# golmschenk/sr-gan

Hardware: AMD Instinct MI355X
Metric: SRGAN train images/sec (G+D step) (higher is better)
Workload: dtype f32; 1 GPU; crowd SRGAN (KnnDenseNetCat D/DNN + DCGenerator) 512x512, batch 16/GPU, dnn_training_step + gan_training_step per step; global_batch=16, image_size=512, schedule=shared-forwards, parallelism=dp1, random_init_weights=True, gradient_penalty=active, launch=eager (Python tape enqueues every kernel), schedule_check=not run: the --full option runs it

## Files before the change

include/srgan_hip.h:

```cpp
#ifndef SRGAN_HIP_H
#define SRGAN_HIP_H

#include <stdint.h>

#ifdef __cplusplus
extern "C" {
#endif

int srgan_version(void);
const char* srgan_build_id(void);
const char* srgan_last_error(void);

#define SRGAN_DTYPE_F32 0x1u
#define SRGAN_DTYPE_BF16 0x2u
#define SRGAN_DTYPE_F16 0x4u
#define SRGAN_FEATURE_FUSED_BNRELU 0x1u
#define SRGAN_FEATURE_SPLITK_WORKSPACE 0x2u
#define SRGAN_FEATURE_LIVE_PROFILE 0x4u
#define SRGAN_FEATURE_BLOCKED16 0x8u
#define SRGAN_FEATURE_BATCHED_SHADOWS 0x10u
#define SRGAN_FEATURE_CROWD_FULL_IMAGE 0x20u
#define SRGAN_FEATURE_IMAGE_BATCHES 0x40u
#define SRGAN_FEATURE_BATCH_NORM_TRAIN 0x80u
typedef struct srgan_capabilities_t {
// ... 31 lines not shown

int srgan_conv2d_bwd_weight(const srgan_conv_desc* desc, const float* x, const float* gy, float* gw, int accumulate,
                            int force_kernel, void* stream);

typedef struct srgan_bn_relu { const float* mean; const float* inv_std; const float* gamma; const float* beta; } srgan_bn_relu;
int srgan_conv2d_bnrelu_supported(const srgan_conv_desc* desc, int pass);
int srgan_conv2d_fwd_bnrelu(const srgan_conv_desc* desc, const float* x, const srgan_bn_relu* bn, const float* w,
                            const float* bias, float* y, void* stream);
int srgan_conv2d_fwd_bnrelu_splits(const srgan_conv_desc* desc);
int srgan_conv2d_fwd_bnrelu_into_zeros(const srgan_conv_desc* desc, const float* x, const srgan_bn_relu* bn, const float* w,
                                       const float* bias, float* y, void* stream);
int srgan_conv2d_bwd_data_bnrelu(const srgan_conv_desc* desc, const float* gy, const float* w, const srgan_bn_relu* bn,
                                 const float* x, float* gx, float* g_gamma, float* g_beta, int accumulate, void* stream);
int srgan_conv2d_bwd_weight_bnrelu(const srgan_conv_desc* desc, const float* x, const srgan_bn_relu* bn, const float* gy,
                                   float* gw, int accumulate, void* stream);
typedef struct srgan_bn_reduce_job {
  int64_t partial_offset;
  int32_t tiles, channels;
  const float* inv_std;
  float* g_gamma;
  float* g_beta;
} srgan_bn_reduce_job;
int64_t srgan_conv2d_bwd_data_bnrelu_tiles(const srgan_conv_desc* desc);
int srgan_conv2d_bwd_data_bnrelu_partials(const srgan_conv_desc* desc, const float* gy, const float* w, const srgan_bn_relu* bn,
                                          const float* x, float* gx, float* partials, int accumulate, void* stream);
int srgan_bn_partial_reduce_batched(const srgan_bn_reduce_job* jobs_device, int32_t count, int32_t max_channels, int32_t max_tiles,
                                    const float* scratch, void* stream);

int srgan_wgrad_group_plan(const srgan_conv_desc* desc, const srgan_bn_relu* bn, int64_t x_offset, int64_t gy_offset, float* gw,
                           int64_t gw_offset, int32_t group_size, int64_t group_weights, int64_t partial_offset, void* job,
// ... 185 lines not shown
```

sr-gan_amd/_lib.py:

```python
import ctypes
import os

from ._build import LIBRARY, source_id

c_float_p = ctypes.c_void_p
i32, i64, f32, vp = ctypes.c_int32, ctypes.c_int64, ctypes.c_float, ctypes.c_void_p


class ConvDesc(ctypes.Structure):
    _fields_ = [(name, i32) for name in ('N', 'C', 'H', 'W', 'K', 'R', 'S', 'stride_h', 'stride_w', 'pad_h', 'pad_w',
                                         'OH', 'OW')] + [('x_batch_stride', i64), ('y_batch_stride', i64), ('compute_dtype', i32)]


class BnRelu(ctypes.Structure):
    _fields_ = [(name, vp) for name in ('mean', 'inv_std', 'gamma', 'beta')]


class BnReduceJob(ctypes.Structure):
    _fields_ = [('partial_offset', i64), ('tiles', i32), ('channels', i32), ('inv_std', vp), ('g_gamma', vp), ('g_beta', vp)]


class Capabilities(ctypes.Structure):
    _fields_ = [('abi_version', i32), ('struct_bytes', i32), ('arch', ctypes.c_char * 16), ('dtypes', ctypes.c_uint32),
                ('features', ctypes.c_uint32), ('workspace_bytes', i64), ('max_tensor_elements', i64)]


SIGNATURES = {
    'srgan_version': ([], ctypes.c_int),
    'srgan_build_id': ([], ctypes.c_char_p),
    'srgan_last_error': ([], ctypes.c_char_p),
    'srgan_conv2d_fwd': ([ctypes.POINTER(ConvDesc), vp, vp, vp, vp, ctypes.c_int, vp], ctypes.c_int),
    'srgan_conv2d_bwd_data': ([ctypes.POINTER(ConvDesc), vp, vp, vp, vp, ctypes.c_int, ctypes.c_int, vp],
                              ctypes.c_int),
    'srgan_conv2d_bwd_weight': ([ctypes.POINTER(ConvDesc), vp, vp, vp, ctypes.c_int, ctypes.c_int, vp], ctypes.c_int),
    'srgan_conv2d_bnrelu_supported': ([ctypes.POINTER(ConvDesc), ctypes.c_int], ctypes.c_int),
    'srgan_conv2d_fwd_bnrelu': ([ctypes.POINTER(ConvDesc), vp, ctypes.POINTER(BnRelu), vp, vp, vp, vp], ctypes.c_int),
    'srgan_conv2d_fwd_bnrelu_into_zeros': ([ctypes.POINTER(ConvDesc), vp, ctypes.POINTER(BnRelu), vp, vp, vp, vp],
                                           ctypes.c_int),
    'srgan_conv2d_fwd_bnrelu_splits': ([ctypes.POINTER(ConvDesc)], ctypes.c_int),
    'srgan_bn_conv_tangent_weights': ([vp, vp, vp, vp, vp, vp, vp, i32, i32, i32, vp], ctypes.c_int),
    'srgan_conv2d_bwd_data_bnrelu': ([ctypes.POINTER(ConvDesc), vp, vp, ctypes.POINTER(BnRelu), vp, vp, vp, vp,
                                      ctypes.c_int, vp], ctypes.c_int),
    'srgan_conv2d_bwd_data_bnrelu_tiles': ([ctypes.POINTER(ConvDesc)], ctypes.c_int64),
    'srgan_conv2d_bwd_data_bnrelu_partials': ([ctypes.POINTER(ConvDesc), vp, vp, ctypes.POINTER(BnRelu), vp, vp, vp,
                                               ctypes.c_int, vp], ctypes.c_int),
    'srgan_bn_partial_reduce_batched': ([vp, i32, i32, i32, vp, vp], ctypes.c_int),
    'srgan_conv2d_bwd_weight_bnrelu': ([ctypes.POINTER(ConvDesc), vp, ctypes.POINTER(BnRelu), vp, vp, ctypes.c_int, vp],
                                       ctypes.c_int),
    'srgan_gemm_f32': ([i32, i32, i32, vp, i64, i64, vp, i64, i64, vp, i64, i64, vp, i32, ctypes.c_int, ctypes.c_int,
                        vp], ctypes.c_int),
    'srgan_gemm': ([i32, i32, i32, vp, i64, i64, vp, i64, i64, vp, i64, i64, vp, i32, ctypes.c_int, ctypes.c_int,
                    ctypes.c_int, vp], ctypes.c_int),
    'srgan_ew_unary': ([ctypes.c_int, vp, vp, i64, f32, f32, vp], ctypes.c_int),
    'srgan_ew_binary': ([ctypes.c_int, vp, vp, vp, i64, f32, vp], ctypes.c_int),
# ... 157 lines not shown
```

sr-gan_amd/csrc/gather_gemm_kernels.hip:

```cpp
#include "common.h"
#include "split_finish.h"
#include "gather_gemm.h"
#include "conv_plan.h"
#include "launchers.h"
#include <stdarg.h>
#include <string.h>
#include <stdlib.h>
#include <atomic>
#include <map>
#include <mutex>
#include <string>
#include <type_traits>
#include <type_traits>
#include <utility>

namespace srgan {

static thread_local char g_error[512] = "";

void set_error(const char* fmt, ...) {
  va_list ap;
  va_start(ap, fmt);
  vsnprintf(g_error, sizeof(g_error), fmt, ap);
  va_end(ap);
// ... 993 lines not shown
    if (pointwise(g)) return use_pointwise(g, g.K, 0) ? 1 : 0;
    return (use_conv3x3(g, g.K, 0) && g.C <= 512) ? 1 : 0;
  }
  if (pass == 1) {
    if ((size_t)g.N * g.H * g.W * g.C / 8 > WORKSPACE_BYTES) return 0;
    if (pointwise(g)) return use_pointwise(g, g.C, 0) ? 1 : 0;
    return (use_conv3x3(g, g.C, 0) && conv3x3_epilogue_supported(g.N, g.K, g.C, g.H, g.W)) ? 1 : 0;
  }
  if (pass == 2) {
    if (pointwise(g)) return pointwise_wgrad_geometry(g) ? 1 : 0;
    return wgrad3x3_geometry(g) ? 1 : 0;
  }
  return 0;
}

static int fwd_bnrelu(const srgan_conv_desc* desc, const float* x, const srgan_bn_relu* bn, const float* w, const float* bias,
                      float* y, int y_state, int* plan_only_split, void* stream) {
  ConvGeom g;
  SRGAN_GEOM(desc, g, "srgan_conv2d_fwd_bnrelu");
  SRGAN_REQUIRE(plan_only_split || (x && w && y && bn_ok(bn)), SRGAN_EINVAL, "srgan_conv2d_fwd_bnrelu pointers");
  SRGAN_REQUIRE(srgan_conv2d_bnrelu_supported(desc, 0), SRGAN_EUNSUPPORTED, "srgan_conv2d_fwd_bnrelu geometry support");
  const float* const coefficients[4] = {bn ? bn->mean : nullptr, bn ? bn->inv_std : nullptr, bn ? bn->gamma : nullptr,
                                        bn ? bn->beta : nullptr};
  if (pointwise(g) && (plan_only_split || ((uintptr_t)w & 15) == 0) &&
      pointwise_ksplit_wanted(g.N, g.C, g.K, g.H * g.W, true)) {
    if (plan_only_split) { *plan_only_split = 1; return SRGAN_OK; }
    return pointwise_ksplit_run(x, g.x_bs, w, bias, y, g.y_bs, g.N, g.C, g.K, g.H * g.W, 0, (hipStream_t)stream,
                                coefficients);
  }
  if (pointwise(g))
// ... 256 lines not shown
```

sr-gan_amd/csrc/launchers.h:

```cpp
#pragma once
#include "common.h"

namespace srgan {

int profile_bracket_begin(hipStream_t stream);
int profile_bracket_end(int slot, hipStream_t stream, int64_t M, int64_t N, int64_t K, int kind, int bm, int bn, int split,
                        int akf = 0, int bkf = 0, int64_t b_unique = 0, int precision = 0);
int profile_bracket_end_bytes(int slot, hipStream_t stream, int64_t M, int64_t N, int64_t K, int kind, int bm, int bn, int split,
                              double bytes, int precision);

struct Conv3Placement { int32_t taps, out_plane, out_sy, out_sx, out_off; };
int conv3x3_splits(int32_t N, int32_t CI, int32_t CO, int32_t H, int32_t W, int precision = 0);
bool conv3x3_epilogue_supported(int32_t N, int32_t CI, int32_t CO, int32_t H, int32_t W);
int64_t conv3x3_epilogue_tiles(int32_t N, int32_t CI, int32_t CO, int32_t H, int32_t W);
int conv3x3_run(const float* in, int64_t in_bs, const float* w, int32_t w_base, int32_t w_so, int32_t w_si, int32_t w_skh,
                int32_t w_skw, const float* bias, float* out, int64_t out_bs, int32_t N, int32_t CI, int32_t CO, int32_t H,
                int32_t W, int accumulate, hipStream_t stream, const float* const* bn = nullptr,
                const BnBackwardEpilogue* epilogue = nullptr, int precision = 0, const Conv3Placement* placement = nullptr);

constexpr int GROUP_OVERSUBSCRIPTION = 4;

int conv3x3_wgrad_run(const float* x, int64_t x_bs, const float* gy, int64_t gy_bs, float* gw, int32_t N, int32_t CI,
                      int32_t CO, int32_t H, int32_t W, int accumulate, hipStream_t stream, const float* const* bn = nullptr,
                      int precision = 0);
// ... 10 lines not shown
                  int* plan_only_split = nullptr);
int64_t pointwise_epilogue_tiles(int32_t N, int32_t HW);
void bn_partial_reduce_run(const float* partial, int tiles, int CO, const float* inv_std, float* g_gamma, float* g_beta,
                           hipStream_t stream);
int bn_partial_reduce_batched_run(const srgan_bn_reduce_job* jobs, int count, int max_channels, int max_tiles,
                                  const float* scratch, hipStream_t stream);

bool pointwise_ring_eligible(const float* in, int64_t in_bs, const float* w, int32_t w_so, int32_t w_si, const float* bias,
                             const float* out, int64_t out_bs, int32_t N, int32_t CI, int32_t CO, int32_t HW, bool fused_pro,
                             const BnBackwardEpilogue* epilogue, int* tile_pixels);
int pointwise_ring_run(const float* in, int64_t in_bs, const float* w, int32_t w_so, int32_t w_si, float* out, int64_t out_bs,
                       int32_t N, int32_t CI, int32_t CO, int32_t HW, int accumulate, hipStream_t stream,
                       const float* const* bn, const BnBackwardEpilogue* epilogue, float* epi_partial, int32_t epi_cols,
                       int tile_pixels, int32_t* rows_done);

bool pointwise_ksplit_wanted(int32_t N, int32_t K, int32_t M, int32_t HW, bool fused_bn);
int pointwise_ksplit_run(const float* in, int64_t in_bs, const float* w, const float* bias, float* out, int64_t out_bs,
                         int32_t N, int32_t K, int32_t M, int32_t HW, int accumulate, hipStream_t stream,
                         const float* const* bn);

bool pointwise_wgrad_enabled();
int pointwise_wgrad_run(const float* x, int64_t x_bs, const float* gy, int64_t gy_bs, float* gw, int32_t N, int32_t CI,
                        int32_t CO, int32_t HW, int accumulate, hipStream_t stream, const float* const* bn = nullptr);
int pointwise_wgrad_group_plan(int64_t x_off, int64_t x_bs, int64_t gy_off, int64_t gy_bs, float* gw, int64_t gw_off, int32_t N, int32_t CI,
                               int32_t CO, int32_t HW, const float* const* bn, int32_t group, int64_t group_weights, int64_t partial_offset,
                               void* job_out, int32_t* grid_x, int32_t* grid_y, int32_t* ragged, int64_t* partial_floats);
int pointwise_wgrad_group_run(const void* jobs, int32_t count, int32_t grid_x, int32_t grid_y, int32_t ragged, int32_t fused_bn,
                              const float* x_base, const float* gy_base, float* gw_base, int64_t flops_mn, int64_t pixels,
                              int64_t elements, int64_t partial_floats, hipStream_t stream);

// ... 22 lines not shown
```

sr-gan_amd/csrc/pointwise.hip:

```cpp
#include "common.h"
#include "launchers.h"
#include "split_finish.h"
#include <stdlib.h>
#include <type_traits>

namespace srgan {

typedef float f32x16 __attribute__((ext_vector_type(16)));

struct PointwiseParams {
  const float* in;
  const float* w;
  float* out;
  const float* bias;
  int32_t N, CI, CO, HW;
  int64_t in_bs, out_bs;
  int32_t w_so, w_si;
  int32_t gpi;
  int32_t tiles_m;
  int32_t xcd_remap;
  int32_t m_base;
  int32_t k_per_split;
  int32_t mode;
  float* split_ws;
// ... 549 lines not shown
  const int profile_slot = profile_bracket_begin(stream);
  p.xcd_remap = (p.tiles_m > 1 && blocks % 8 == 0) ? 1 : 0;
  const dim3 grid((unsigned)blocks, (unsigned)split, 1);
  if (mi == 2) launch_pointwise<2>(p, grid, stream);
  else launch_pointwise<1>(p, grid, stream);
  if (p.epi_partial && !epilogue->partial_out)
    bn_partial_reduce_run(p.epi_partial, (int)col_blocks, CO, p.bn_inv, epilogue->g_gamma, epilogue->g_beta, stream);
  const int status = launch_status();
  const int64_t pixels = (int64_t)N * HW;
  const int64_t b_elements = (int64_t)CI * pixels + (epilogue ? (int64_t)CO * pixels * (p.mode == 1 ? 2 : 1) : 0) +
                             ((!epilogue && p.mode == 1) ? (int64_t)CO * pixels : 0);
  profile_bracket_end(profile_slot, stream, CO, pixels, CI, 3, mi * 32, 128, split, 0, 0, b_elements);
  return status;
}

}
```

sr-gan_amd/csrc/pointwise_ring.hip:

```cpp
#include <atomic>
#include "common.h"
#include "launchers.h"
#include "lds_dma.h"
#include <stdlib.h>
#include <type_traits>

namespace srgan {

typedef float f32x16 __attribute__((ext_vector_type(16)));
typedef float f32x4 __attribute__((ext_vector_type(4)));
typedef float f32x2 __attribute__((ext_vector_type(2)));

struct RingParams {
  const float* in;
  const float* w;
  float* out;
  int32_t N, CI, CO, HW;
  int64_t in_bs, out_bs;
  int32_t w_ld;
  int32_t bpi;
  int32_t tiles_m;
  int32_t xcd_remap;
  int32_t mode;
  const float* bn_mean; const float* bn_inv; const float* bn_gamma; const float* bn_beta;
  const float* epi_x; int64_t epi_x_bs;
  float* epi_partial; int32_t epi_cols;
};

template <int STAGES, int NI, bool A_KCONTIG, int FUSE>
__global__ __launch_bounds__(256, 2) void pointwise_ring_kernel(const RingParams p) {
  constexpr int BK = 32;
  constexpr int A_BYTES = 128 * BK * 4, RB = 128 * NI, B_BYTES = BK * RB, C_BYTES = FUSE == 1 ? 4 * 512 : 0;
  constexpr int STAGE_BYTES = A_BYTES + B_BYTES + C_BYTES;
  constexpr int QA = 4, QB = NI, RPI = 1024 / RB;
  constexpr int PER_STAGE = QA + QB + (FUSE == 1 ? 2 : 0);
  static_assert(FUSE != 2 || NI == 4, "the epilogue's partial sums are per 128-pixel block");
  extern __shared__ __attribute__((aligned(16))) char smem[];
  const int tid = threadIdx.x, lane = tid & 63, l31 = lane & 31, lhi = lane >> 5;
  const int wave = __builtin_amdgcn_readfirstlane(tid >> 6);
  int bid = (int)blockIdx.x;
  if (p.xcd_remap) bid = (bid & 7) * ((int)gridDim.x >> 3) + (bid >> 3);
  const int tm = bid % p.tiles_m, cb = bid / p.tiles_m;
  const int n = cb / p.bpi, pix0 = (cb - n * p.bpi) * (32 * NI);
  const int m0 = tm * 128;
  const uint32_t lds0 = ring_lds_address(smem);
  const int nst = p.CI / BK;

  const char* in_block = (const char*)(p.in + (int64_t)n * p.in_bs + pix0);
  const int b_row = lane / (RB / 16), b_col = lane % (RB / 16);
  const uint32_t b_lane = (uint32_t)(b_row * p.HW + 4 * b_col) * 4u;
  uint32_t a_lane[QA];
  if (A_KCONTIG) {
#pragma unroll
    for (int q = 0; q < QA; ++q) {
      const int br = lane >> 4, sp = lane & 15;
      const int bank_row = 16 * wave + 4 * q + br;
      const int s = sp ^ (bank_row & 15);
      a_lane[q] = (uint32_t)(min(m0 + 2 * bank_row + (s >> 3), p.CO - 1) * p.w_ld + 4 * (s & 7)) * 4u;
    }
  } else {
#pragma unroll
    for (int q = 0; q < QA; ++q)
      a_lane[q] = (uint32_t)(((wave * QA + q) * 2 + lhi) * p.w_ld + min(m0 + 4 * l31, p.CO - 4)) * 4u;
  }
  const bool active = m0 + 32 * wave < p.CO;
  const float* c_lane0 = (lhi ? p.bn_inv : p.bn_mean) + l31;
  const float* c_lane1 = (lhi ? p.bn_beta : p.bn_gamma) + l31;
  auto issue = [&](int stage) {
    const uint32_t slot = lds0 + (uint32_t)(stage % STAGES) * STAGE_BYTES;
    const char* xb = in_block + (int64_t)(stage * BK + wave * QB * RPI) * p.HW * 4;
#pragma unroll
    for (int q = 0; q < QB; ++q)
      ring_glds16(xb + (int64_t)(q * RPI) * p.HW * 4, b_lane, slot + A_BYTES + (uint32_t)((wave * QB + q) * RPI) * RB);
    const char* wb = (const char*)p.w + (A_KCONTIG ? (int64_t)stage * BK * 4 : (int64_t)stage * BK * p.w_ld * 4);
#pragma unroll
    for (int q = 0; q < QA; ++q)
      ring_glds16(wb, a_lane[q], slot + (A_KCONTIG ? (uint32_t)(4096 * wave + 1024 * q) : (uint32_t)((wave * QA + q) * 1024)));
    if (FUSE == 1) {
      ring_glds4(c_lane0 + stage * BK, slot + A_BYTES + B_BYTES + wave * 512);
      ring_glds4(c_lane1 + stage * BK, slot + A_BYTES + B_BYTES + wave * 512 + 256);
    }
  };

  uint32_t a_read[4];
  if (A_KCONTIG) {
    const int row = 32 * wave + l31, bank_row = row >> 1;
#pragma unroll
    for (int g = 0; g < 4; ++g) a_read[g] = (uint32_t)(bank_row * 256 + ((((row & 1) * 8 + 2 * g + lhi) ^ (bank_row & 15)) * 16));
  } else {
#pragma unroll
    for (int g = 0; g < 4; ++g) a_read[g] = (uint32_t)((8 * g + 4 * lhi) * 512 + (32 * wave + l31) * 4);
  }
  const uint32_t b_read = (uint32_t)(A_BYTES + (4 * lhi) * RB + l31 * (4 * NI));
  const uint32_t c_read = (uint32_t)(A_BYTES + B_BYTES + wave * 512 + 16 * lhi);

  f32x16 acc[NI];
#pragma unroll
  for (int ni = 0; ni < NI; ++ni)
#pragma unroll
    for (int r = 0; r < 16; ++r) acc[ni][r] = 0.f;

  struct Group { float a[4]; float b[4][NI]; f32x4 mean, inv, gamma, beta; };
  auto load_group = [&](Group& f, const char* slot, int g) {
    if (A_KCONTIG) {
      const f32x4 v = *reinterpret_cast<const f32x4*>(slot + a_read[g]);
      f.a[0] = v.x; f.a[1] = v.y; f.a[2] = v.z; f.a[3] = v.w;
    } else {
#pragma unroll
      for (int q = 0; q < 4; ++q) f.a[q] = *reinterpret_cast<const float*>(slot + a_read[g] + q * 512);
    }
#pragma unroll
    for (int q = 0; q < 4; ++q) {
      if constexpr (NI == 4) {
        const f32x4 v = *reinterpret_cast<const f32x4*>(slot + b_read + (8 * g + q) * RB);
        f.b[q][0] = v.x; f.b[q][1] = v.y; f.b[q][2] = v.z; f.b[q][3] = v.w;
      } else if constexpr (NI == 2) {
        const f32x2 v = *reinterpret_cast<const f32x2*>(slot + b_read + (8 * g + q) * RB);
        f.b[q][0] = v.x; f.b[q][1] = v.y;
      } else {
        f.b[q][0] = *reinterpret_cast<const float*>(slot + b_read + (8 * g + q) * RB);
      }
    }
    if (FUSE == 1) {
      f.mean = *reinterpret_cast<const f32x4*>(slot + c_read + 32 * g);
      f.inv = *reinterpret_cast<const f32x4*>(slot + c_read + 128 + 32 * g);
      f.gamma = *reinterpret_cast<const f32x4*>(slot + c_read + 256 + 32 * g);
      f.beta = *reinterpret_cast<const f32x4*>(slot + c_read + 384 + 32 * g);
    }
  };
  auto compute_group = [&](const Group& f) {
#pragma unroll
    for (int q = 0; q < 4; ++q) {
      float b[NI];
      if (FUSE == 1) {
        float ca, cb;
        bn_coefficients(f.mean[q], f.inv[q], f.gamma[q], f.beta[q], ca, cb);
#pragma unroll
        for (int ni = 0; ni < NI; ++ni) b[ni] = fmaxf(fmaf(f.b[q][ni], ca, cb), 0.f);
      } else {
#pragma unroll
        for (int ni = 0; ni < NI; ++ni) b[ni] = f.b[q][ni];
      }
#pragma unroll
      for (int ni = 0; ni < NI; ++ni) acc[ni] = __builtin_amdgcn_mfma_f32_32x32x2f32(f.a[q], b[ni], acc[ni], 0, 0, 0);
    }
  };

  const int64_t row0 = m0 + 32 * wave + 4 * lhi;
  float* out_lane = p.out + (int64_t)n * p.out_bs + row0 * p.HW + pix0 + NI * l31;
  const float* x_lane = FUSE == 2 ? p.epi_x + (int64_t)n * p.epi_x_bs + row0 * p.HW + pix0 + 4 * l31 : nullptr;
  f32x4 xs[FUSE == 2 ? 16 : 1], olds[FUSE == 2 ? 16 : 1];
  const bool prefetch = FUSE == 2 && STAGES == 2 && nst >= 3 && active;
  const bool accumulate = p.mode == 1;

  for (int s = 0; s < STAGES - 1 && s < nst; ++s) issue(s);
  for (int t = 0; t < nst; ++t) {
    if (FUSE == 2 && prefetch && (t == 1 || (t == 2 && accumulate))) ring_wait_and_barrier<16>();
    else if (nst - 1 - t >= STAGES - 2) ring_wait_and_barrier<PER_STAGE * (STAGES - 2)>();
    else ring_wait_and_barrier<0>();
    if (t + STAGES - 1 < nst) issue(t + STAGES - 1);
    if constexpr (FUSE == 2) {
      if (prefetch && t == 0) {
#pragma unroll
        for (int r = 0; r < 16; ++r) xs[r] = *reinterpret_cast<const f32x4*>(x_lane + (int64_t)((r & 3) + 8 * (r >> 2)) * p.HW);
      }
      if (prefetch && t == 1 && accumulate) {
#pragma unroll
        for (int r = 0; r < 16; ++r) olds[r] = *reinterpret_cast<const f32x4*>(out_lane + (int64_t)((r & 3) + 8 * (r >> 2)) * p.HW);
      }
    }
    if (!active) continue;
    const char* slot = smem + (t % STAGES) * STAGE_BYTES;
    Group f0, f1;
    load_group(f0, slot, 0);
    load_group(f1, slot, 1);
    compute_group(f0);
    load_group(f0, slot, 2);
    compute_group(f1);
    load_group(f1, slot, 3);
    compute_group(f0);
    compute_group(f1);
  }

  if constexpr (FUSE == 2) {
    __syncthreads();
    float* table = reinterpret_cast<float*>(smem);
    if (tid < 128) {
      const int o = min(m0 + tid, p.CO - 1);
      const float mu = p.bn_mean[o];
      float a, b;
      bn_coefficients(mu, p.bn_inv[o], p.bn_gamma[o], p.bn_beta[o], a, b);
      table[tid * 4 + 0] = a; table[tid * 4 + 1] = b; table[tid * 4 + 2] = mu;
    }
    __syncthreads();
    if (!active) return;
    const bool sums_wanted = p.epi_partial != nullptr;
// ... 27 lines not shown
            const float plain = half_wave_sum((v.x + v.y) + (v.z + v.w));
            const float centred = half_wave_sum((v.x * (x.x - t.z) + v.y * (x.y - t.z)) + (v.z * (x.z - t.z) + v.w * (x.w - t.z)));
            if (l31 == 31) {
              partial[local] = plain;
              partial[(int64_t)p.epi_cols * p.CO + local] = centred;
            }
          }
        }
        __builtin_amdgcn_sched_barrier(0);
      }
    };
    if (accumulate) rows(std::true_type{});
    else rows(std::false_type{});
    return;
  }
  if (!active) return;
  if (p.mode == 1) {
    float previous[16][NI];
#pragma unroll
    for (int r = 0; r < 16; ++r) {
      const float* src = out_lane + (int64_t)((r & 3) + 8 * (r >> 2)) * p.HW;
      if constexpr (NI == 4) {
        const f32x4 v = *reinterpret_cast<const f32x4*>(src);
        previous[r][0] = v.x; previous[r][1] = v.y; previous[r][2] = v.z; previous[r][3] = v.w;
      } else if constexpr (NI == 2) {
        const f32x2 v = *reinterpret_cast<const f32x2*>(src);
        previous[r][0] = v.x; previous[r][1] = v.y;
      } else {
        previous[r][0] = *src;
      }
// ... 43 lines not shown
  constexpr int narrow_below = 512, slim_below = 384, min_blocks = 192;
  const int64_t tiles = (int64_t)N * ((CO + 127) / 128);
  int pixels = 128;
  if (epilogue) pixels = 128;
  else if (HW % 128 != 0 || tiles * (HW / 128) < narrow_below) pixels = 64;
  if (!epilogue && (HW % 64 != 0 || (pixels == 64 && tiles * (HW / 64) < slim_below))) pixels = 32;
  if (tiles * (HW / pixels) < min_blocks) return false;
  (void)fused_pro;
  *tile_pixels = pixels;
  return true;
}

template <int NI, bool A_KCONTIG, int FUSE>
static int launch_ring(const RingParams& p, unsigned blocks, hipStream_t stream) {
  constexpr int STAGES = 2;
  constexpr int bytes = STAGES * (128 * 32 * 4 + 32 * 128 * NI + (FUSE == 1 ? 2048 : 0));
  auto kernel = pointwise_ring_kernel<STAGES, NI, A_KCONTIG, FUSE>;
  static std::atomic<uint64_t> configured_devices{0};
  int device = 0;
  SRGAN_HIP(hipGetDevice(&device));
  const uint64_t bit = (uint64_t)1 << (device & 63);
  if (!(configured_devices.load(std::memory_order_acquire) & bit)) {
    SRGAN_HIP(hipFuncSetAttribute((const void*)kernel, hipFuncAttributeMaxDynamicSharedMemorySize, bytes));
    configured_devices.fetch_or(bit, std::memory_order_release);
  }
  hipLaunchKernelGGL(kernel, dim3(blocks), dim3(256), bytes, stream, p);
  return launch_status();
}

int pointwise_ring_run(const float* in, int64_t in_bs, const float* w, int32_t w_so, int32_t w_si, float* out, int64_t out_bs,
                       int32_t N, int32_t CI, int32_t CO, int32_t HW, int accumulate, hipStream_t stream,
// ... 21 lines not shown
  const unsigned grid = (unsigned)blocks;
  const int fuse = epilogue ? 2 : (bn ? 1 : 0);
  if (fuse == 2) return k_contiguous ? launch_ring<4, true, 2>(p, grid, stream) : launch_ring<4, false, 2>(p, grid, stream);
  if (tile_pixels == 32) {
    if (fuse == 1) return k_contiguous ? launch_ring<1, true, 1>(p, grid, stream) : launch_ring<1, false, 1>(p, grid, stream);
    return k_contiguous ? launch_ring<1, true, 0>(p, grid, stream) : launch_ring<1, false, 0>(p, grid, stream);
  }
  if (tile_pixels == 64) {
    if (fuse == 1) return k_contiguous ? launch_ring<2, true, 1>(p, grid, stream) : launch_ring<2, false, 1>(p, grid, stream);
    return k_contiguous ? launch_ring<2, true, 0>(p, grid, stream) : launch_ring<2, false, 0>(p, grid, stream);
  }
  if (fuse == 1) return k_contiguous ? launch_ring<4, true, 1>(p, grid, stream) : launch_ring<4, false, 1>(p, grid, stream);
  return k_contiguous ? launch_ring<4, true, 0>(p, grid, stream) : launch_ring<4, false, 0>(p, grid, stream);
}

}
```

sr-gan_amd/fused.py:

```python

import torch

from . import _lib
from . import functional as F
from .tape import Var, Node, grad_enabled, incoming_gradient_is_exclusive, at_sweep_end
from .nn import parameter_var


ENABLED = True
POOL_FIRST = True
PROLOGUE = True
EPILOGUE = True
WGRAD_STREAM = False
_side_streams = {}


def _side_stream(device, main=None):
    key = (str(device), main.cuda_stream if main is not None else 0)
    if key not in _side_streams:
        _side_streams[key] = torch.cuda.Stream(device=device)
    return _side_streams[key]


def _launch_on_side_stream(device, tensors, launch):
# ... 59 lines not shown
            max_channels, max_tiles = max(max_channels, channels), max(max_tiles, tiles)
        offsets.append(entry)
    if not jobs:
        return None
    import ctypes
    table = (_lib.BnReduceJob * len(jobs))(*jobs)
    host = torch.frombuffer(bytearray(bytes(table)), dtype=torch.uint8)
    plan = dict(key=key, offsets=offsets, total=total, count=len(jobs), max_channels=max_channels, max_tiles=max_tiles,
                jobs=host.to(device), keep=[norm._inverse_std() for layer in layers for norm in (layer.norm1, layer.norm2)])
    plans[key] = plan
    return plan


GROUPED_WGRAD = True
GROUPED_TANGENT_LIMIT = 4096 << 20


def _wgrad_plan(layers, n, c0, h, w, growth, buffer_bs, device, tangent=None):
    import ctypes
    key = (n, c0, h, w, str(device), tangent is not None, layers[0].conv1.weight.grad.data_ptr(),
           layers[-1].conv2.weight.grad.data_ptr())
    plans = layers[0].__dict__.setdefault('_srgan_wgrad_plans', {})
    if key in plans:
        return plans[key]
    lib = _lib.library()
    width, hw = layers[0].conv1.out_channels, h * w
    plan = {'keep': []}
    u1_offsets, u1_at = [], 0
    for index in range(len(layers)):
        u1_offsets.append(u1_at)
# ... 307 lines not shown
        if GROUPED_WGRAD and want_params and g_b1_all is not None:
            grouped = _wgrad_plan(layers, n, c0, h, w, growth, buffer_bs, device, tangent)
            if grouped is not None and 4 * grouped['u1_total'] > GROUPED_TANGENT_LIMIT:
                grouped = None
        u1_all = _empty((grouped['u1_total'],), device) if grouped is not None else None
        u2_all = _empty((len(layers), n, layers[0].conv1.out_channels, h, w), device) if grouped is not None else None
        for index, layer in enumerate(layers):
            g_b1, b1 = kept[index]
            cin = c0 + index * growth
            width = layer.conv1.out_channels
            mean1, inv1, gamma1, beta1 = norm_pointers(layer.norm1)
            mean2, inv2, gamma2, beta2 = norm_pointers(layer.norm2)
            at1, at2 = tangent['offsets'][index]
            desc1 = _desc(n, cin, h, w, width, 1, 1, 1, 0)
            desc2 = _desc(n, width, h, w, growth, 3, 3, 1, 1, 0, buffer_bs)
            u1 = _empty((n, cin, h, w), device) if grouped is None else None
            u1_ptr = u1.data_ptr() if grouped is None else _ptr(u1_all, grouped['u1_offsets'][index])
            F._call('srgan_bn_act_bwd', vbuf.data_ptr(), buffer.data_ptr(), mean1, inv1, gamma1, beta1, 1, u1_ptr,
                    None, None, n, cin, hw, buffer_bs, buffer_bs, 0, 0, 1, stream)
            if want_params and grouped is None:
                F._call('srgan_conv2d_bwd_weight', desc1, u1_ptr, g_b1.data_ptr(), _ptr(q_all, at1), 1, 0, stream)
            b1_tangent = _empty(b1.shape, device)
            F._call('srgan_conv2d_fwd', desc1, u1_ptr, _ptr(scaled_all, at1), None, b1_tangent.data_ptr(), 0, stream)
            del u1
            u2 = u2_all[index] if grouped is not None else _empty(b1.shape, device)
            F._call('srgan_bn_act_bwd', b1_tangent.data_ptr(), b1.data_ptr(), mean2, inv2, gamma2, beta2, 1, u2.data_ptr(),
                    None, None, n, width, hw, 0, 0, 0, 0, 1, stream)
            if want_params and grouped is None:
                F._call('srgan_conv2d_bwd_weight', desc2, u2.data_ptr(), _ptr(gbuf, cin * hw), _ptr(q_all, at2), 1, 0, stream)
            F._call('srgan_conv2d_fwd', desc2, u2.data_ptr(), _ptr(scaled_all, at2), None, _ptr(vbuf, cin * hw), 0, stream)
            kept[index] = None
        def run_parameter_part(on):
            if grouped is not None:
                _run_wgrad_group(grouped[1], 1, False, u1_all, g_b1_all, q_all, on)
                _run_wgrad_group(grouped[3], 3, False, u2_all, gbuf, q_all, on)
            F._call('srgan_bn_conv_tangent_weights_grouped', tangent['table'].data_ptr(), tangent['count'],
                    tangent['max_inner'], tangent['max_co'], None, q_all.data_ptr(), on)
        if want_params and grouped is not None and WGRAD_STREAM and not torch.cuda.is_current_stream_capturing():
            _launch_on_side_stream(device, (u1_all, u2_all, g_b1_all, gbuf, q_all, scaled_all), run_parameter_part)
        elif want_params:
# ... 45 lines not shown
                    norm.bias.grad.data_ptr() if want_params else None, 0, stream)
            if needs[0]:
                gx = Var(gx_data)
                if recorded:
                    gx.requires_grad = True
                    gx.node = Node((g,) + tuple(parameter_vars), lambda v, needs2: double_backward(v, needs2, g),
                                   'bn_relu_conv_backward')
        return (gx,) + (None,) * len(parameter_vars)

    def double_backward(v, needs2, g):
        if grad_enabled():
            raise NotImplementedError('third-order differentiation of the fused norm -> relu -> conv')
        stream = F._stream()
        want_params = any(needs2[1:])
        inv, mean = norm._inverse_std()
        u = _empty((n, cin, h, w), device)
        F._call('srgan_bn_act_bwd', v.data.data_ptr(), x.data.data_ptr(), mean.data.data_ptr(), inv.data.data_ptr(),
                norm.weight.data_ptr(), norm.bias.data_ptr(), 1, u.data_ptr(), None, None, n, cin, hw, 0, 0, 0, 0, 1, stream)
        q = None
        if want_params:
            q = _zeros(tuple(conv.weight.shape), device)
            F._call('srgan_conv2d_bwd_weight', desc, u.data_ptr(), g.data.data_ptr(), q.data_ptr(), 1, 0, stream)
        scaled = _empty(conv.weight.shape, device)
        F._call('srgan_bn_conv_tangent_weights', conv.weight.data_ptr(), q.data_ptr() if want_params else None,
                inv.data.data_ptr(), norm.weight.data_ptr(), scaled.data_ptr(),
                conv.weight.grad.data_ptr() if want_params else None,
                norm.weight.grad.data_ptr() if want_params else None, cout, cin, 1, stream)
        tangent = None
        if needs2[0]:
            tangent = _empty((n, cout, h, w), device)
# ... 7 lines not shown
```

Baseline: 88.21 images/s.

## Fuse BN-ReLU tangent masking into pointwise conv for gradient-penalty double backward

Adds a FUSE==3 variant of the pointwise ring GEMM kernel. It applies the input BN-ReLU mask to the tangent inside the prologue, can write the masked tangent out for the weight gradient, and applies the output BN-ReLU mask in the epilogue. The dense-block and bn_relu_conv double-backward paths now use it instead of separate bn_act_bwd, conv and bn_act_bwd launches. This removes several elementwise kernels and the intermediate round trips through memory. In exchange it loads a second activation tile per stage (more LDS, possibly lower occupancy) and splits the tangent-weights call into two.

```diff
diff --git a/include/srgan_hip.h b/include/srgan_hip.h
--- a/include/srgan_hip.h
+++ b/include/srgan_hip.h
@@ -69,6 +69,10 @@
                                  const float* x, float* gx, float* g_gamma, float* g_beta, int accumulate, void* stream);
 int srgan_conv2d_bwd_weight_bnrelu(const srgan_conv_desc* desc, const float* x, const srgan_bn_relu* bn, const float* gy,
                                    float* gw, int accumulate, void* stream);
+int srgan_conv2d_masked_tangent_supported(const srgan_conv_desc* desc);
+int srgan_conv2d_masked_tangent(const srgan_conv_desc* desc, const float* v, const float* x, const srgan_bn_relu* bn_in,
+                                const float* w, const float* ref, const srgan_bn_relu* bn_out, float* masked_out, float* y,
+                                void* stream);
 typedef struct srgan_bn_reduce_job {
   int64_t partial_offset;
   int32_t tiles, channels;
diff --git a/sr-gan_amd/_lib.py b/sr-gan_amd/_lib.py
--- a/sr-gan_amd/_lib.py
+++ b/sr-gan_amd/_lib.py
@@ -38,6 +38,9 @@
     'srgan_conv2d_fwd_bnrelu_into_zeros': ([ctypes.POINTER(ConvDesc), vp, ctypes.POINTER(BnRelu), vp, vp, vp, vp],
                                            ctypes.c_int),
     'srgan_conv2d_fwd_bnrelu_splits': ([ctypes.POINTER(ConvDesc)], ctypes.c_int),
+    'srgan_conv2d_masked_tangent_supported': ([ctypes.POINTER(ConvDesc)], ctypes.c_int),
+    'srgan_conv2d_masked_tangent': ([ctypes.POINTER(ConvDesc), vp, vp, ctypes.POINTER(BnRelu), vp, vp, ctypes.POINTER(BnRelu), vp,
+                                     vp, vp], ctypes.c_int),
     'srgan_bn_conv_tangent_weights': ([vp, vp, vp, vp, vp, vp, vp, i32, i32, i32, vp], ctypes.c_int),
     'srgan_conv2d_bwd_data_bnrelu': ([ctypes.POINTER(ConvDesc), vp, vp, ctypes.POINTER(BnRelu), vp, vp, vp, vp,
                                       ctypes.c_int, vp], ctypes.c_int),
diff --git a/sr-gan_amd/csrc/gather_gemm_kernels.hip b/sr-gan_amd/csrc/gather_gemm_kernels.hip
--- a/sr-gan_amd/csrc/gather_gemm_kernels.hip
+++ b/sr-gan_amd/csrc/gather_gemm_kernels.hip
@@ -1031,6 +1031,29 @@
   return 0;
 }
 
+int srgan_conv2d_masked_tangent_supported(const srgan_conv_desc* desc) {
+  ConvGeom g;
+  if (desc && desc->compute_dtype != 0) return 0;
+  if (!to_geom(desc, g) || geom_largest_extent(g) >= ((int64_t)1 << 31) || !pointwise(g)) return 0;
+  return pointwise_masked_tangent_geometry(g.N, g.C, g.K, g.H * g.W, g.x_bs, g.y_bs, nullptr) ? 1 : 0;
+}
+
+int srgan_conv2d_masked_tangent(const srgan_conv_desc* desc, const float* v, const float* x, const srgan_bn_relu* bn_in,
+                                const float* w, const float* ref, const srgan_bn_relu* bn_out, float* masked_out, float* y,
+                                void* stream) {
+  ConvGeom g;
+  SRGAN_GEOM(desc, g, "srgan_conv2d_masked_tangent");
+  SRGAN_REQUIRE(v && x && w && y && bn_ok(bn_in), SRGAN_EINVAL, "srgan_conv2d_masked_tangent pointers");
+  SRGAN_REQUIRE((ref == nullptr) == (bn_out == nullptr) && (!bn_out || bn_ok(bn_out)), SRGAN_EINVAL,
+                "srgan_conv2d_masked_tangent output mask (ref and bn_out: both or neither)");
+  SRGAN_REQUIRE(srgan_conv2d_masked_tangent_supported(desc), SRGAN_EUNSUPPORTED, "srgan_conv2d_masked_tangent geometry support");
+  const float* const in_vectors[4] = {bn_in->mean, bn_in->inv_std, bn_in->gamma, bn_in->beta};
+  const float* const out_vectors[4] = {bn_out ? bn_out->mean : nullptr, bn_out ? bn_out->inv_std : nullptr,
+                                       bn_out ? bn_out->gamma : nullptr, bn_out ? bn_out->beta : nullptr};
+  return pointwise_masked_tangent_run(v, x, g.x_bs, in_vectors, w, ref, out_vectors, masked_out, y, g.y_bs, g.N, g.C, g.K,
+                                      g.H * g.W, (hipStream_t)stream);
+}
+
 static int fwd_bnrelu(const srgan_conv_desc* desc, const float* x, const srgan_bn_relu* bn, const float* w, const float* bias,
                       float* y, int y_state, int* plan_only_split, void* stream) {
   ConvGeom g;
diff --git a/sr-gan_amd/csrc/launchers.h b/sr-gan_amd/csrc/launchers.h
--- a/sr-gan_amd/csrc/launchers.h
+++ b/sr-gan_amd/csrc/launchers.h
@@ -48,6 +48,15 @@
                        const float* const* bn, const BnBackwardEpilogue* epilogue, float* epi_partial, int32_t epi_cols,
                        int tile_pixels, int32_t* rows_done);
 
+bool pointwise_masked_tangent_geometry(int32_t N, int32_t CI, int32_t CO, int32_t HW, int64_t in_bs, int64_t out_bs,
+                                       int* tile_pixels);
+int pointwise_masked_tangent_ring_run(const float* in, const float* mask_x, int64_t in_bs, const float* const* bn_in, const float* w,
+                                      const float* ref, const float* const* bn_out, float* masked_out, float* out, int64_t out_bs,
+                                      int32_t N, int32_t CI, int32_t CO, int32_t HW, int tile_pixels, hipStream_t stream);
+int pointwise_masked_tangent_run(const float* in, const float* mask_x, int64_t in_bs, const float* const* bn_in, const float* w,
+                                 const float* ref, const float* const* bn_out, float* masked_out, float* out, int64_t out_bs,
+                                 int32_t N, int32_t CI, int32_t CO, int32_t HW, hipStream_t stream);
+
 bool pointwise_ksplit_wanted(int32_t N, int32_t K, int32_t M, int32_t HW, bool fused_bn);
 int pointwise_ksplit_run(const float* in, int64_t in_bs, const float* w, const float* bias, float* out, int64_t out_bs,
                          int32_t N, int32_t K, int32_t M, int32_t HW, int accumulate, hipStream_t stream,
diff --git a/sr-gan_amd/csrc/pointwise.hip b/sr-gan_amd/csrc/pointwise.hip
--- a/sr-gan_amd/csrc/pointwise.hip
+++ b/sr-gan_amd/csrc/pointwise.hip
@@ -587,4 +587,25 @@
   return status;
 }
 
-}
+int pointwise_masked_tangent_run(const float* in, const float* mask_x, int64_t in_bs, const float* const* bn_in, const float* w,
+                                 const float* ref, const float* const* bn_out, float* masked_out, float* out, int64_t out_bs,
+                                 int32_t N, int32_t CI, int32_t CO, int32_t HW, hipStream_t stream) {
+  int tile_pixels = 0;
+  SRGAN_REQUIRE(pointwise_masked_tangent_geometry(N, CI, CO, HW, in_bs, out_bs, &tile_pixels), SRGAN_EUNSUPPORTED,
+                "masked tangent geometry");
+  SRGAN_REQUIRE(((((uintptr_t)in | (uintptr_t)mask_x | (uintptr_t)w | (uintptr_t)out | (uintptr_t)ref | (uintptr_t)masked_out)) & 15) == 0,
+                SRGAN_EINVAL, "masked tangent: 16-byte aligned tensors");
+  const int profile_slot = profile_bracket_begin(stream);
+  const int status = pointwise_masked_tangent_ring_run(in, mask_x, in_bs, bn_in, w, ref, bn_out, masked_out, out, out_bs, N, CI, CO,
+                                                       HW, tile_pixels, stream);
+  if (status != SRGAN_OK) {
+    profile_bracket_end(profile_slot, stream, 0, 0, 0, 13, 128, tile_pixels, 1);
+    return status;
+  }
+  const int64_t pixels = (int64_t)N * HW;
+  const int64_t b_elements = (int64_t)CI * pixels * (masked_out ? 3 : 2) + (ref ? (int64_t)CO * pixels : 0);
+  profile_bracket_end(profile_slot, stream, CO, pixels, CI, 13, 128, tile_pixels, 1, 0, 0, b_elements);
+  return SRGAN_OK;
+}
+
+}
diff --git a/sr-gan_amd/csrc/pointwise_ring.hip b/sr-gan_amd/csrc/pointwise_ring.hip
--- a/sr-gan_amd/csrc/pointwise_ring.hip
+++ b/sr-gan_amd/csrc/pointwise_ring.hip
@@ -25,16 +25,21 @@
   const float* bn_mean; const float* bn_inv; const float* bn_gamma; const float* bn_beta;
   const float* epi_x; int64_t epi_x_bs;
   float* epi_partial; int32_t epi_cols;
+  const float* mask_x; float* masked_out;
+  const float* out_bn_mean; const float* out_bn_inv; const float* out_bn_gamma; const float* out_bn_beta;
 };
 
 template <int STAGES, int NI, bool A_KCONTIG, int FUSE>
 __global__ __launch_bounds__(256, 2) void pointwise_ring_kernel(const RingParams p) {
   constexpr int BK = 32;
-  constexpr int A_BYTES = 128 * BK * 4, RB = 128 * NI, B_BYTES = BK * RB, C_BYTES = FUSE == 1 ? 4 * 512 : 0;
-  constexpr int STAGE_BYTES = A_BYTES + B_BYTES + C_BYTES;
+  constexpr bool BN_PRO = FUSE == 1 || FUSE == 3;
+  constexpr int A_BYTES = 128 * BK * 4, RB = 128 * NI, B_BYTES = BK * RB, X_BYTES = FUSE == 3 ? B_BYTES : 0;
+  constexpr int C_BYTES = BN_PRO ? 4 * 512 : 0;
+  constexpr int STAGE_BYTES = A_BYTES + B_BYTES + X_BYTES + C_BYTES;
   constexpr int QA = 4, QB = NI, RPI = 1024 / RB;
-  constexpr int PER_STAGE = QA + QB + (FUSE == 1 ? 2 : 0);
+  constexpr int PER_STAGE = QA + QB + (FUSE == 3 ? QB : 0) + (BN_PRO ? 2 : 0);
   static_assert(FUSE != 2 || NI == 4, "the epilogue's partial sums are per 128-pixel block");
+  static_assert(FUSE != 3 || NI <= 2, "two activation tiles per stage: the 128-pixel tile would leave one workgroup per CU");
   extern __shared__ __attribute__((aligned(16))) char smem[];
   const int tid = threadIdx.x, lane = tid & 63, l31 = lane & 31, lhi = lane >> 5;
   const int wave = __builtin_amdgcn_readfirstlane(tid >> 6);
@@ -47,6 +52,7 @@
   const int nst = p.CI / BK;
 
   const char* in_block = (const char*)(p.in + (int64_t)n * p.in_bs + pix0);
+  const char* mask_block = FUSE == 3 ? (const char*)(p.mask_x + (int64_t)n * p.in_bs + pix0) : nullptr;
   const int b_row = lane / (RB / 16), b_col = lane % (RB / 16);
   const uint32_t b_lane = (uint32_t)(b_row * p.HW + 4 * b_col) * 4u;
   uint32_t a_lane[QA];
@@ -72,13 +78,19 @@
 #pragma unroll
     for (int q = 0; q < QB; ++q)
       ring_glds16(xb + (int64_t)(q * RPI) * p.HW * 4, b_lane, slot + A_BYTES + (uint32_t)((wave * QB + q) * RPI) * RB);
+    if constexpr (FUSE == 3) {
+      const char* mb = mask_block + (int64_t)(stage * BK + wave * QB * RPI) * p.HW * 4;
+#pragma unroll
+      for (int q = 0; q < QB; ++q)
+        ring_glds16(mb + (int64_t)(q * RPI) * p.HW * 4, b_lane, slot + A_BYTES + B_BYTES + (uint32_t)((wave * QB + q) * RPI) * RB);
+    }
     const char* wb = (const char*)p.w + (A_KCONTIG ? (int64_t)stage * BK * 4 : (int64_t)stage * BK * p.w_ld * 4);
 #pragma unroll
     for (int q = 0; q < QA; ++q)
       ring_glds16(wb, a_lane[q], slot + (A_KCONTIG ? (uint32_t)(4096 * wave + 1024 * q) : (uint32_t)((wave * QA + q) * 1024)));
-    if (FUSE == 1) {
-      ring_glds4(c_lane0 + stage * BK, slot + A_BYTES + B_BYTES + wave * 512);
-      ring_glds4(c_lane1 + stage * BK, slot + A_BYTES + B_BYTES + wave * 512 + 256);
+    if (BN_PRO) {
+      ring_glds4(c_lane0 + stage * BK, slot + A_BYTES + B_BYTES + X_BYTES + wave * 512);
+      ring_glds4(c_lane1 + stage * BK, slot + A_BYTES + B_BYTES + X_BYTES + wave * 512 + 256);
     }
   };
 
@@ -92,7 +104,7 @@
     for (int g = 0; g < 4; ++g) a_read[g] = (uint32_t)((8 * g + 4 * lhi) * 512 + (32 * wave + l31) * 4);
   }
   const uint32_t b_read = (uint32_t)(A_BYTES + (4 * lhi) * RB + l31 * (4 * NI));
-  const uint32_t c_read = (uint32_t)(A_BYTES + B_BYTES + wave * 512 + 16 * lhi);
+  const uint32_t c_read = (uint32_t)(A_BYTES + B_BYTES + X_BYTES + wave * 512 + 16 * lhi);
 
   f32x16 acc[NI];
 #pragma unroll
@@ -100,7 +112,7 @@
 #pragma unroll
     for (int r = 0; r < 16; ++r) acc[ni][r] = 0.f;
 
-  struct Group { float a[4]; float b[4][NI]; f32x4 mean, inv, gamma, beta; };
+  struct Group { float a[4]; float b[4][NI]; float x[FUSE == 3 ? 4 : 1][NI]; f32x4 mean, inv, gamma, beta; };
   auto load_group = [&](Group& f, const char* slot, int g) {
     if (A_KCONTIG) {
       const f32x4 v = *reinterpret_cast<const f32x4*>(slot + a_read[g]);
@@ -121,18 +133,46 @@
         f.b[q][0] = *reinterpret_cast<const float*>(slot + b_read + (8 * g + q) * RB);
       }
     }
-    if (FUSE == 1) {
+    if constexpr (FUSE == 3) {
+#pragma unroll
+      for (int q = 0; q < 4; ++q) {
+        if constexpr (NI == 2) {
+          const f32x2 v = *reinterpret_cast<const f32x2*>(slot + B_BYTES + b_read + (8 * g + q) * RB);
+          f.x[q][0] = v.x; f.x[q][1] = v.y;
+        } else {
+          f.x[q][0] = *reinterpret_cast<const float*>(slot + B_BYTES + b_read + (8 * g + q) * RB);
+        }
+      }
+    }
+    if (BN_PRO) {
       f.mean = *reinterpret_cast<const f32x4*>(slot + c_read + 32 * g);
       f.inv = *reinterpret_cast<const f32x4*>(slot + c_read + 128 + 32 * g);
       f.gamma = *reinterpret_cast<const f32x4*>(slot + c_read + 256 + 32 * g);
       f.beta = *reinterpret_cast<const f32x4*>(slot + c_read + 384 + 32 * g);
     }
   };
-  auto compute_group = [&](const Group& f) {
+  const bool store_masked = FUSE == 3 && p.masked_out != nullptr && tm == 0;
+  float* masked_lane = FUSE == 3 ? p.masked_out + ((int64_t)n * p.CI + 4 * lhi) * p.HW + pix0 + NI * l31 : nullptr;
+  auto compute_group = [&](const Group& f, int t, int g) {
 #pragma unroll
     for (int q = 0; q < 4; ++q) {
       float b[NI];
-      if (FUSE == 1) {
+      if constexpr (FUSE == 3) {
+        float ca, cb;
+        bn_coefficients(f.mean[q], f.inv[q], f.gamma[q], f.beta[q], ca, cb);
+#pragma unroll
+        for (int ni = 0; ni < NI; ++ni) b[ni] = fmaf(f.x[q][ni], ca, cb) > 0.f ? f.b[q][ni] : 0.f;
+        if (store_masked && g == wave) {
+          float* dst = masked_lane + (int64_t)(t * BK + 8 * g + q) * p.HW;
+          if constexpr (NI == 2) {
+            f32x2 v;
+            v.x = b[0]; v.y = b[1];
+            *reinterpret_cast<f32x2*>(dst) = v;
+          } else {
+            *dst = b[0];
+          }
+        }
+      } else if (FUSE == 1) {
         float ca, cb;
         bn_coefficients(f.mean[q], f.inv[q], f.gamma[q], f.beta[q], ca, cb);
 #pragma unroll
@@ -156,6 +196,7 @@
   for (int s = 0; s < STAGES - 1 && s < nst; ++s) issue(s);
   for (int t = 0; t < nst; ++t) {
     if (FUSE == 2 && prefetch && (t == 1 || (t == 2 && accumulate))) ring_wait_and_barrier<16>();
+    else if (FUSE == 3 && STAGES == 2 && store_masked && t > 0) ring_wait_and_barrier<4>();
     else if (nst - 1 - t >= STAGES - 2) ring_wait_and_barrier<PER_STAGE * (STAGES - 2)>();
     else ring_wait_and_barrier<0>();
     if (t + STAGES - 1 < nst) issue(t + STAGES - 1);
@@ -174,12 +215,12 @@
     Group f0, f1;
     load_group(f0, slot, 0);
     load_group(f1, slot, 1);
-    compute_group(f0);
+    compute_group(f0, t, 0);
     load_group(f0, slot, 2);
-    compute_group(f1);
+    compute_group(f1, t, 1);
     load_group(f1, slot, 3);
-    compute_group(f0);
-    compute_group(f1);
+    compute_group(f0, t, 2);
+    compute_group(f1, t, 3);
   }
 
   if constexpr (FUSE == 2) {
@@ -237,6 +278,47 @@
     else rows(std::false_type{});
     return;
   }
+  if constexpr (FUSE == 3) {
+    if (p.epi_x) {
+      __syncthreads();
+      float* table = reinterpret_cast<float*>(smem);
+      if (tid < 128) {
+        const int o = min(m0 + tid, p.CO - 1);
+        float a, b;
+        bn_coefficients(p.out_bn_mean[o], p.out_bn_inv[o], p.out_bn_gamma[o], p.out_bn_beta[o], a, b);
+        table[tid * 2 + 0] = a; table[tid * 2 + 1] = b;
+      }
+      __syncthreads();
+      if (!active) return;
+      const float* ref_lane = p.epi_x + (int64_t)n * p.epi_x_bs + row0 * p.HW + pix0 + NI * l31;
+      float ref[16][NI];
+#pragma unroll
+      for (int r = 0; r < 16; ++r) {
+        const float* src = ref_lane + (int64_t)((r & 3) + 8 * (r >> 2)) * p.HW;
+        if constexpr (NI == 2) {
+          const f32x2 v = *reinterpret_cast<const f32x2*>(src);
+          ref[r][0] = v.x; ref[r][1] = v.y;
+        } else {
+          ref[r][0] = *src;
+        }
+      }
+#pragma unroll
+      for (int r = 0; r < 16; ++r) {
+        const int local = (r & 3) + 8 * (r >> 2);
+        const f32x2 t = *reinterpret_cast<const f32x2*>(table + (32 * wave + 4 * lhi + local) * 2);
+        float* dst = out_lane + (int64_t)local * p.HW;
+        if constexpr (NI == 2) {
+          f32x2 v;
+          v.x = fmaf(ref[r][0], t.x, t.y) > 0.f ? acc[0][r] : 0.f;
+          v.y = fmaf(ref[r][1], t.x, t.y) > 0.f ? acc[1][r] : 0.f;
+          __builtin_nontemporal_store(v, reinterpret_cast<f32x2*>(dst));
+        } else {
+          __builtin_nontemporal_store(fmaf(ref[r][0], t.x, t.y) > 0.f ? acc[0][r] : 0.f, dst);
+        }
+      }
+      return;
+    }
+  }
   if (!active) return;
   if (p.mode == 1) {
     float previous[16][NI];
@@ -310,7 +392,7 @@
 template <int NI, bool A_KCONTIG, int FUSE>
 static int launch_ring(const RingParams& p, unsigned blocks, hipStream_t stream) {
   constexpr int STAGES = 2;
-  constexpr int bytes = STAGES * (128 * 32 * 4 + 32 * 128 * NI + (FUSE == 1 ? 2048 : 0));
+  constexpr int bytes = STAGES * (128 * 32 * 4 + 32 * 128 * NI * (FUSE == 3 ? 2 : 1) + (FUSE == 1 || FUSE == 3 ? 2048 : 0));
   auto kernel = pointwise_ring_kernel<STAGES, NI, A_KCONTIG, FUSE>;
   static std::atomic<uint64_t> configured_devices{0};
   int device = 0;
@@ -362,4 +444,38 @@
   return k_contiguous ? launch_ring<4, true, 0>(p, grid, stream) : launch_ring<4, false, 0>(p, grid, stream);
 }
 
-}
+bool pointwise_masked_tangent_geometry(int32_t N, int32_t CI, int32_t CO, int32_t HW, int64_t in_bs, int64_t out_bs,
+                                       int* tile_pixels) {
+  if (CO < 128 || CO % 32 != 0 || CI % 32 != 0 || CI < 32 || HW % 32 != 0 || (in_bs & 3) || (out_bs & 3)) return false;
+  if (in_bs < (int64_t)CI * HW || out_bs < (int64_t)CO * HW) return false;
+  if (pointwise_ksplit_wanted(N, CI, CO, HW, false)) return false;
+  constexpr int slim_below = 384;
+  const int64_t tiles = (int64_t)N * ((CO + 127) / 128);
+  const int pixels = (HW % 64 == 0 && tiles * (HW / 64) >= slim_below) ? 64 : 32;
+  if (tiles * (HW / pixels) >= ((int64_t)1 << 31)) return false;
+  if (tile_pixels) *tile_pixels = pixels;
+  return true;
+}
+
+int pointwise_masked_tangent_ring_run(const float* in, const float* mask_x, int64_t in_bs, const float* const* bn_in, const float* w,
+                                      const float* ref, const float* const* bn_out, float* masked_out, float* out, int64_t out_bs,
+                                      int32_t N, int32_t CI, int32_t CO, int32_t HW, int tile_pixels, hipStream_t stream) {
+  RingParams p;
+  p.in = in; p.w = w; p.out = out;
+  p.N = N; p.CI = CI; p.CO = CO; p.HW = HW; p.in_bs = in_bs; p.out_bs = out_bs;
+  p.w_ld = CI;
+  p.tiles_m = (CO + 127) / 128;
+  p.bpi = HW / tile_pixels;
+  p.mode = 0;
+  p.bn_mean = bn_in[0]; p.bn_inv = bn_in[1]; p.bn_gamma = bn_in[2]; p.bn_beta = bn_in[3];
+  p.epi_x = ref; p.epi_x_bs = (int64_t)CO * HW; p.epi_partial = nullptr; p.epi_cols = 0;
+  p.mask_x = mask_x; p.masked_out = masked_out;
+  p.out_bn_mean = ref ? bn_out[0] : nullptr; p.out_bn_inv = ref ? bn_out[1] : nullptr;
+  p.out_bn_gamma = ref ? bn_out[2] : nullptr; p.out_bn_beta = ref ? bn_out[3] : nullptr;
+  const int64_t blocks = (int64_t)N * p.bpi * p.tiles_m;
+  p.xcd_remap = (p.tiles_m > 1 && blocks % 8 == 0) ? 1 : 0;
+  if (tile_pixels == 64) return launch_ring<2, true, 3>(p, (unsigned)blocks, stream);
+  return launch_ring<1, true, 3>(p, (unsigned)blocks, stream);
+}
+
+}
diff --git a/sr-gan_amd/fused.py b/sr-gan_amd/fused.py
--- a/sr-gan_amd/fused.py
+++ b/sr-gan_amd/fused.py
@@ -97,6 +97,7 @@
 
 GROUPED_WGRAD = True
 GROUPED_TANGENT_LIMIT = 4096 << 20
+MASKED_TANGENT = True
 
 
 def _wgrad_plan(layers, n, c0, h, w, growth, buffer_bs, device, tangent=None):
@@ -434,6 +435,20 @@
             at1, at2 = tangent['offsets'][index]
             desc1 = _desc(n, cin, h, w, width, 1, 1, 1, 0)
             desc2 = _desc(n, width, h, w, growth, 3, 3, 1, 1, 0, buffer_bs)
+            u2 = u2_all[index] if grouped is not None else _empty(b1.shape, device)
+            desc1_views = _desc(n, cin, h, w, width, 1, 1, 1, 0, buffer_bs, 0)
+            if MASKED_TANGENT and lib.srgan_conv2d_masked_tangent_supported(desc1_views):
+                u1 = _empty((n, cin, h, w), device) if grouped is None and want_params else None
+                u1_ptr = _ptr(u1_all, grouped['u1_offsets'][index]) if grouped is not None else (u1.data_ptr() if want_params else None)
+                F._call('srgan_conv2d_masked_tangent', desc1_views, vbuf.data_ptr(), buffer.data_ptr(), bn_struct(layer.norm1),
+                        _ptr(scaled_all, at1), b1.data_ptr(), bn_struct(layer.norm2), u1_ptr, u2.data_ptr(), stream)
+                if want_params and grouped is None:
+                    F._call('srgan_conv2d_bwd_weight', desc1, u1_ptr, g_b1.data_ptr(), _ptr(q_all, at1), 1, 0, stream)
+                    F._call('srgan_conv2d_bwd_weight', desc2, u2.data_ptr(), _ptr(gbuf, cin * hw), _ptr(q_all, at2), 1, 0, stream)
+                del u1
+                F._call('srgan_conv2d_fwd', desc2, u2.data_ptr(), _ptr(scaled_all, at2), None, _ptr(vbuf, cin * hw), 0, stream)
+                kept[index] = None
+                continue
             u1 = _empty((n, cin, h, w), device) if grouped is None else None
             u1_ptr = u1.data_ptr() if grouped is None else _ptr(u1_all, grouped['u1_offsets'][index])
             F._call('srgan_bn_act_bwd', vbuf.data_ptr(), buffer.data_ptr(), mean1, inv1, gamma1, beta1, 1, u1_ptr,
@@ -443,7 +458,6 @@
             b1_tangent = _empty(b1.shape, device)
             F._call('srgan_conv2d_fwd', desc1, u1_ptr, _ptr(scaled_all, at1), None, b1_tangent.data_ptr(), 0, stream)
             del u1
-            u2 = u2_all[index] if grouped is not None else _empty(b1.shape, device)
             F._call('srgan_bn_act_bwd', b1_tangent.data_ptr(), b1.data_ptr(), mean2, inv2, gamma2, beta2, 1, u2.data_ptr(),
                     None, None, n, width, hw, 0, 0, 0, 0, 1, stream)
             if want_params and grouped is None:
@@ -519,6 +533,21 @@
         stream = F._stream()
         want_params = any(needs2[1:])
         inv, mean = norm._inverse_std()
+        if MASKED_TANGENT and lib.srgan_conv2d_masked_tangent_supported(desc) and (needs2[0] or want_params):
+            scaled = _empty(conv.weight.shape, device)
+            F._call('srgan_bn_conv_tangent_weights', conv.weight.data_ptr(), None, inv.data.data_ptr(), norm.weight.data_ptr(),
+                    scaled.data_ptr(), None, None, cout, cin, 1, stream)
+            u = _empty((n, cin, h, w), device) if want_params else None
+            tangent = _empty((n, cout, h, w), device)
+            F._call('srgan_conv2d_masked_tangent', desc, v.data.data_ptr(), x.data.data_ptr(), bn_struct(), scaled.data_ptr(),
+                    None, None, u.data_ptr() if want_params else None, tangent.data_ptr(), stream)
+            if want_params:
+                q = _zeros(tuple(conv.weight.shape), device)
+                F._call('srgan_conv2d_bwd_weight', desc, u.data_ptr(), g.data.data_ptr(), q.data_ptr(), 1, 0, stream)
+                F._call('srgan_bn_conv_tangent_weights', conv.weight.data_ptr(), q.data_ptr(), inv.data.data_ptr(),
+                        norm.weight.data_ptr(), None, conv.weight.grad.data_ptr(), norm.weight.grad.data_ptr(), cout, cin, 1,
+                        stream)
+            return (Var(tangent) if needs2[0] else None,) + (None,) * len(parameter_vars)
         u = _empty((n, cin, h, w), device)
         F._call('srgan_bn_act_bwd', v.data.data_ptr(), x.data.data_ptr(), mean.data.data_ptr(), inv.data.data_ptr(),
                 norm.weight.data_ptr(), norm.bias.data_ptr(), 1, u.data_ptr(), None, None, n, cin, hw, 0, 0, 0, 0, 1, stream)
```

Measured after the change: 88.52 images/s (median of 6 runs). Within noise of the previous version (+0.4%).
